# dnbaker/dashing2

Hardware: AMD Instinct MI355X
Metric: all-pairs sketch comparison throughput (pairs/s) (higher is better)
Workload: dtype u64

## Files before the change

dashing2_amd/capi.py:

```python
import ctypes as C
import os
import subprocess

import numpy as np

_HERE = os.path.dirname(os.path.abspath(__file__))
LIB_PATH = os.environ.get("D2G_LIB") or os.path.join(_HERE, "libd2g.so")
_lib = None

SIMILARITY, CONTAINMENT, SYMMETRIC_CONTAINMENT, POISSON_LLR, INTERSECTION, UNION_SIZE = range(6)
CMP_AUTO, CMP_DIRECT, CMP_BITSLICE, CMP_PLANES = 0, 1, 2, 3
BITSLICE_OPS_PER_GROUP_EXTRA = 1


TIME_K1, TIME_K2, TIME_K2PREP, TIME_K3, TIME_K0 = 2, 4, 8, 16, 32
TIME_KNN = 64
TIME_DEDUP = 128
TIME_FILTER = 256
TIME_KSET = 512
TIME_SCREEN = 1024


class D2GError(RuntimeError):
    def __init__(self, status, detail=""):
        self.status = status
        name = lib().d2g_strerror(status).decode() if _lib is not None else str(status)
        super().__init__(f"d2g error {status} ({name}){': ' + detail if detail else ''}")


def build(jobs=8):
    subprocess.check_call(["make", "-s", f"-j{jobs}", "-C", os.path.join(_HERE, "csrc")])
    return LIB_PATH

# ... 1323 lines not shown
                lib().d2g_cmp_set_destroy(self._h)
            self._h = None

    __del__ = close

    def export_operand_dev(self, planes_out_ptr, meta_out_ptr, stream=None):
        self.ctx._check(lib().d2g_cmp_set_export_operand_dev(self.ctx._h, self._h, planes_out_ptr, meta_out_ptr, stream))

    def update_dev(self, dev_ptr, stream=None):
        self.ctx._check(lib().d2g_cmp_set_update_dev(self.ctx._h, self._h, dev_ptr, stream))

    def status(self, stream=None):
        self.ctx._check(lib().d2g_cmp_set_status(self.ctx._h, self._h, stream))

    def sparse_info(self, stream=None):
        a = np.zeros(4, np.uint32)
        self.ctx._check(lib().d2g_cmp_set_sparse_info(self.ctx._h, self._h, stream, a.ctypes.data))
        return sparse_info_dict(a)

    def sparse_detail(self, stream=None):
        a = np.zeros(10, np.uint64)
        self.ctx._check(lib().d2g_cmp_set_sparse_detail(self.ctx._h, self._h, stream, a.ctypes.data))
        return {"looked": bool(a[0]), "looked_dense": bool(a[1]), "entries": int(a[2]), "family_pairs": int(a[3]), "shared_values": int(a[4]),
                "planes": int(a[5]), "binned": bool(a[6]), "bin_cshift": int(a[7]), "schedule": "merged" if a[8] else "classic", "prepare_kernels": int(a[9])}

    def fill_detail(self):
        a = np.zeros(4, np.uint64)
        self.ctx._check(lib().d2g_cmp_set_fill_detail(self.ctx._h, self._h, a.ctypes.data))
        return {"announced": int(a[0]), "rank": int(a[1]), "riders": int(a[2]), "launch": int(a[3])}

    def debug_pairs(self, cap=1 << 24, stream=None):
        buf = np.empty(cap, np.uint64)
        roots = np.empty(self.N, np.uint32)
        n = _sz()
        self.ctx._check(lib().d2g_cmp_set_debug_pairs(self.ctx._h, self._h, stream, buf.ctypes.data, cap, C.byref(n), roots.ctypes.data))
        e = buf[:n.value]
        e = e[e != np.uint64(0xFFFFFFFFFFFFFFFF)]
        return np.stack([(e & np.uint64(0xFFFFFFFF)).astype(np.uint32), (e >> np.uint64(32)).astype(np.uint32)], axis=1), roots

    def planes(self, stream=None):
        md, nb, mean = C.c_uint(), _int(), _f32()
        self.ctx._check(lib().d2g_cmp_set_planes(self.ctx._h, self._h, stream, C.byref(md), C.byref(nb), C.byref(mean)))
        return int(md.value), int(nb.value), float(mean.value)

    def eqcount_ut_dev(self, out_dev_ptr, r0=0, r1=None, stream=None):
        r1 = self.N if r1 is None else r1
        self.ctx._check(lib().d2g_cmp_eqcount_ut_dev(self.ctx._h, self._h, r0, r1, out_dev_ptr, stream))
# ... 260 lines not shown
```

dashing2_amd/csrc/d2g_internal.h:

```cpp
#pragma once
#include "../../include/d2g.h"
#include <hip/hip_runtime.h>
#include <cstdio>
#include <memory>
#include <string>
#include <utility>

#include <vector>
struct d2g_ctx;
int d2g_hip_status(d2g_ctx *ctx, hipError_t e, const char *what);

template <class T, bool Pinned> class d2g_owned {
    T *p_ = nullptr; size_t cap_ = 0;
public:
    d2g_owned() = default;
    d2g_owned(d2g_owned &&o) noexcept : p_(o.p_), cap_(o.cap_) { o.p_ = nullptr; o.cap_ = 0; }
    d2g_owned &operator=(d2g_owned &&o) noexcept { if (this != &o) { reset(); p_ = o.p_; cap_ = o.cap_; o.p_ = nullptr; o.cap_ = 0; } return *this; }
    ~d2g_owned() { reset(); }
    void reset() { if (p_) (void)(Pinned ? hipHostFree(p_) : hipFree(p_)); p_ = nullptr; cap_ = 0; }
    int alloc(d2g_ctx *ctx, size_t n, const char *what, unsigned flags = hipHostMallocDefault) {
        reset();
        const hipError_t e = Pinned ? hipHostMalloc((void **)&p_, n * sizeof(T), flags) : hipMalloc((void **)&p_, n * sizeof(T));
        if (e != hipSuccess) p_ = nullptr; else cap_ = n;
        return d2g_hip_status(ctx, e, what);
// ... 27 lines not shown
};

struct d2g_evlog {
    std::vector<d2g_event> a, b;
};

struct d2g_tuning {
    std::vector<std::pair<std::string, std::string>> kv;
    const char *get(const char *name) const {
        for (const auto &p : kv) if (p.first == name) return p.second.c_str();
        return nullptr;
    }
};
void d2g_tuning_load(d2g_tuning &t);
struct d2g_k2_tuning {
    bool sparse = true;
    size_t min_n = 8192;
    int link = 1;
    double tile_frac = 0.35;
    int olink = 1;
    int emit_big = 0;
    int ride = 127;
    int rank_share = 35;
    int merge = 1;
    int remember = 1;
    size_t long_list = 786432;
    int predict = 1;
    int list_form = 0;
    size_t list_div = 8;
    bool sort = true;
    int tagbits_max = 31;
    int id16 = 1;
    int nsplit_req = 0;
};
d2g_k2_tuning d2g_k2_tuning_resolve(const d2g_tuning &t);
std::string d2g_k2_tuning_json(const d2g_ctx *ctx);
uint64_t d2g_k2_tuning_hash(const d2g_ctx *ctx);

constexpr int K3_MAXBBITS = 12;
constexpr int K3_ROUND_KEYS = 1400;
constexpr int K3_TARGET = 1024;
constexpr int K3_L1BITS = 8;
constexpr uint64_t K3_SPLIT_MIN = 4 * 1400;
struct d2g_k3_tuning {
    bool compact = false;
    bool light = true;
    uint32_t l1bits = K3_L1BITS;
// ... 91 lines not shown
```

dashing2_amd/csrc/d2g_k2.h:

```cpp
#pragma once
#include "d2g_internal.h"

#include <algorithm>

struct SpRider { uint32_t *out; size_t cnt; const uint32_t *vsrc; uint32_t vimm, own, piece0; };
constexpr SpRider SP_NO_RIDER{nullptr, 0, nullptr, 0u, 0xFFFFFFFFu, 0u};
constexpr int SP_FILL_PER_THREAD = 8, SP_FILL_THREADS = 256;
inline size_t sp_fill_pieces(size_t cnt) { return div_up<size_t>(cnt / 4 + 1, (size_t)SP_FILL_THREADS * SP_FILL_PER_THREAD); }
#ifndef D2G_SP_RW_M_LINK0
#define D2G_SP_RW_M_LINK0 8
#endif
#ifndef D2G_SP_RW_M_PLANES
#define D2G_SP_RW_M_PLANES 5
#endif
constexpr unsigned SP_RW_PLAN = 6, SP_RW_FLATTEN = 5, SP_RW_COUNT = 5, SP_RW_ATTACH = 5, SP_RW_SCAN = 8, SP_RW_ALL = 35;
constexpr unsigned SP_RW_M_LINK0 = D2G_SP_RW_M_LINK0, SP_RW_M_PLANES = D2G_SP_RW_M_PLANES;
constexpr int BS_RANK_THREADS = 1024, BS_RANK_PF = 12;
constexpr uint32_t SP_RANK_FILL_PER_WG = (uint32_t)(BS_RANK_PF * BS_RANK_THREADS * 16 / (SP_FILL_THREADS * SP_FILL_PER_THREAD * 16));
static_assert(SP_RANK_FILL_PER_WG * SP_FILL_THREADS * SP_FILL_PER_THREAD == BS_RANK_PF * BS_RANK_THREADS, "the rank kernel's stores of one workgroup are whole pieces");

struct SpInit {
    uint32_t *label = nullptr, *ones = nullptr, *zero = nullptr;
    uint32_t n = 0, owords = 0, zwords = 0;
};
// ... 37 lines not shown
        next += n;
        *grid = own + n;
        return r;
    }
};

struct SpFilled {
    uint32_t *out = nullptr;
    size_t cnt = 0;
    size_t pieces = 0;
    const uint32_t *src = nullptr;
    bool by_riders = false;
    void set_early(uint32_t *o, size_t n, const uint32_t *s) { out = o; cnt = n; pieces = (size_t)-1; src = s; by_riders = false; }
    void set_by_riders(const SpAnnounced &a) { out = a.out; cnt = a.cnt; pieces = a.next; src = a.vsrc; by_riders = true; }
    size_t done_for(const uint32_t *o, size_t n, const uint32_t *s, size_t npieces) const { return (out == o && cnt == n && src == s) ? std::min(pieces, npieces) : 0; }
    void void_after_prepare() { if (by_riders) out = nullptr; }
    void clear() { out = nullptr; }
};

enum SpMappedWord : uint32_t { SP_MW_GAVEUP = 0, SP_MW_LIST_LEN = 1, SP_MW_SUMS = 2, SP_MW_TICKET = 6, SP_MW_WORDS = 16 };

struct SpDecision {
    unsigned prepares = 0; bool skipped = false;
    bool merged = false; unsigned kernels = 0;
    int skip_cached = -1;
    bool sample_pending = false; uint32_t sample_ticket = 0;
    bool pred_valid = false, pred_dense = false; double pred_entries = 0, pred_family_pairs = 0;
    bool big = true;
    bool looked = false, looked_dense = false; uint32_t samp_sums[4] = {0, 0, 0, 0};
    uint64_t fill_announced = 0, fill_rank = 0, fill_carried = 0;
};

struct SpState {
    unsigned sp_launch = 0;
    d2g_dev<uint32_t> d_stream_s;
    d2g_dev<uint32_t> d_sperm;
    d2g_dev<uint32_t> d_sinv;
    d2g_dev<uint32_t> d_label;
    d2g_dev<uint32_t> d_owner;
    size_t owner_stride = 0;
    d2g_dev<uint32_t> d_segend;
    d2g_dev<uint32_t> d_posseg;
    d2g_dev<uint32_t> d_hint;
    d2g_dev<uint32_t> d_spz;
    size_t spz_words = 0;
    uint32_t *d_lcnt = nullptr;
    uint32_t *d_gbm = nullptr;
// ... 97 lines not shown
```

dashing2_amd/csrc/d2g_k2_bitslice.hip:

```cpp
#include "d2g_internal.h"
#include "d2g_k2.h"
#include "d2g_k2_shape.h"
#include <chrono>
#include <cstring>
#include <algorithm>
#include <vector>

namespace {

typedef uint32_t u32x16 __attribute__((ext_vector_type(16)));
typedef u32x16 __attribute__((aligned(4))) u32x16_u;
constexpr uint32_t BS_EMPTY = 0xFFFFFFFFu;

constexpr uint32_t BS_DUP = 0x80000000u;
constexpr uint32_t BS_UNIQ = 0x80000000u;
constexpr uint32_t BS_PENDING = 0x40000000u;
constexpr int BS_LOG_TLDS_MAX = 15;
template <typename IdT> struct BsId;
template <> struct BsId<uint32_t> { static constexpr uint32_t UNIQ = BS_UNIQ; static constexpr int UBIT = 31; };
template <> struct BsId<uint16_t> { static constexpr uint32_t UNIQ = 0x8000u; static constexpr int UBIT = 15; };
constexpr size_t BS_ID16_MAX_N = ((size_t(1) << BS_LOG_TLDS_MAX) * 2) / 3;
static_assert(BS_ID16_MAX_N / 2 < BsId<uint16_t>::UNIQ, "16-bit ids: the highest rank (N / 2) must stay below the unique flag");
static_assert((size_t(1) << BS_LOG_TLDS_MAX) - 1 <= 0xFFFFu, "16-bit ids: the general single-partition kernel parks a table slot in ids[] between its two loops");

// ... 437 lines not shown
        uint32_t mx = 0;
        for (uint32_t x = 0; x < 32; ++x) mx = max(mx, d2s[perm_s[(uint32_t)g * 32 + x]]);
        meta[g] = mx + 1;
        if (ex_meta) ex_meta[g] = mx + 1;
    }
}

__global__ __launch_bounds__(BS_PLAN_THREADS) void bs_colplan_kernel(BsPlanArgs pa, SpRider rider) {
    SP_RIDE_OR_WORK(rider);
    extern __shared__ __attribute__((aligned(16))) uint32_t plan_lds[];
    bs_colplan_body<BS_PLAN_THREADS>(pa, bs_plan_lds(plan_lds, (uint32_t)pa.ntb * 32u));
}

constexpr int BS_FORM_STREAM = 1, BS_FORM_EXCHANGE = 2;
constexpr size_t BS_SLACK = 64;
struct BsPlanesArgs {
    const void *ids; size_t N, Npad; uint32_t *planes, *stream; size_t Nstride; int nbits_cap; const uint32_t *meta; int forms;
    const uint32_t *perm, *colcnt, *sperm;
};
BsPlanesArgs planes_args_of(const d2g_cmp_set *set, uint32_t *planes, int forms) {
    return BsPlanesArgs{set->d_ids.get(), set->N, set->Npad, planes, set->d_stream, set->Nstride, set->nbits_cap, set->d_meta, forms, set->d_perm, set->d_colcnt, nullptr};
}
template <bool SPLIT, typename IdT = uint32_t>
__device__ __forceinline__ void bs_planes_body(const BsPlanesArgs &a, size_t bx, size_t tb) {
    static_assert(!SPLIT || sizeof(IdT) == 4, "bs_planes_body: split ranks are 32-bit ids");
    constexpr int UBIT = BsId<IdT>::UBIT;
    const IdT *__restrict__ ids = static_cast<const IdT *>(a.ids);
    const uint32_t *__restrict__ meta = a.meta, *__restrict__ perm = a.perm, *__restrict__ colcnt = a.colcnt, *__restrict__ sperm = a.sperm;
    uint32_t *__restrict__ planes = a.planes, *__restrict__ stream = a.stream;
    const size_t N = a.N, Npad = a.Npad, Nstride = a.Nstride;
    const int nbits_cap = a.nbits_cap, forms = a.forms;
    const size_t jpos = bx * 256 + threadIdx.x;
    const size_t slot = (forms & BS_FORM_STREAM) ? stream_slot_wave(meta, (int)tb) : 0;
    if (jpos >= Nstride) return;
    const size_t j = sperm ? (size_t)sperm[jpos] : jpos;
    const int nbits = live_planes(meta, (int)tb);
    typedef const u32x16_u __attribute__((address_space(4))) *slots_ptr;
    const u32x16_u pa = *(slots_ptr)(uintptr_t)(perm + tb * 32), pb = *(slots_ptr)(uintptr_t)(perm + tb * 32 + 16);
    uint32_t id[32];
#pragma unroll
    for (int x = 0; x < 32; ++x) {
        const uint32_t t = x < 16 ? pa[x] : pb[x - 16];
        const bool real = t != BS_NOCOL && j < N;
        uint32_t w = real ? ids[(size_t)t * Npad + j] : 0u;
        if (SPLIT && real && !(w >> 31)) w = (w & BS_RANK_MASK) + colcnt[(size_t)t * BS_CC_STRIDE + (w >> BS_SPLIT_SHIFT)];
        id[x] = w;
    }
    uint32_t u = 0;
#pragma unroll
    for (int x = 0; x < 32; ++x) u |= (id[x] >> UBIT) << x;
    uint32_t *dst = planes + tb * (size_t)(nbits_cap + 1) * Nstride + jpos;
    const bool ex = forms & BS_FORM_EXCHANGE, st = forms & BS_FORM_STREAM;
    uint32_t *sdst = st ? stream + slot * 2 * Nstride + jpos : nullptr;
    for (int b = 0; b < nbits; ++b) {
        uint32_t w = 0;
// ... 307 lines not shown
        const int logTl = set->logT < BS_LOG_TLDS_MAX ? set->logT : BS_LOG_TLDS_MAX;
        const size_t lds = (size_t(1) << logTl) * sizeof(uint32_t);
        const bool id16 = set->id_bits == 16;
        D2G_CHECK(ctx, !(multi && id16), "bitslice: the multi-partition rank kernel with 16-bit ids");
        void (*kern)(const uint64_t *, size_t, size_t, uint32_t, int, void *, uint32_t *, uint32_t *, int, uint32_t, int, uint32_t *, size_t, SpRider, uint32_t) = bs_rank_kernel<false, false>;
        const bool fast = !multi && N <= (size_t)BS_RANK_PF * BS_RANK_THREADS;
        if (multi) kern = bs_rank_kernel<true, false>;
        else if (fast) kern = id16 ? bs_rank_kernel<false, true, uint16_t> : bs_rank_kernel<false, true>;
        else if (id16) kern = bs_rank_kernel<false, false, uint16_t>;
        if (lds > 48 * 1024)
            D2G_HIP(ctx, hipFuncSetAttribute((const void *)kern, hipFuncAttributeMaxDynamicSharedMemorySize, (int)lds));
        if (nsplit > 1) D2G_HIP(ctx, hipMemsetAsync(set->d_ids, 0, S * Npad * sizeof(uint32_t), s));
        const bool look = sparse_path && sp_sample_due(ctx, set);
        SpRider rank_fill = SP_NO_RIDER; uint32_t rank_n = 0;
        if (sparse_path && fast && !look && sp->announced.riding() < SP_SIDE_FILL_PIECES)
            rank_fill = sp->announced.take_first((unsigned)ctx->k2.rank_share, (uint64_t)SP_RANK_FILL_PER_WG * S, &rank_n);
        D2G_CHECK(ctx, rank_n <= (uint64_t)SP_RANK_FILL_PER_WG * S * nsplit, "bitslice: the rank kernel's share of the fill does not fit its grid");
        if (sp) sp->dec.fill_rank = rank_n;
        hipLaunchKernelGGL(kern, dim3((unsigned)(S * nsplit)), dim3(BS_RANK_THREADS), lds, s, set->d_cols, N, Npad, set->T, set->logT,
                           (void *)set->d_ids.get(), set->d_colcnt, set->d_meta + set->ntb, ctx->k2.tagbits_max, (uint32_t)S, nsplit,
                           (sp && nsplit == 1) ? sp->d_owner.get() : (uint32_t *)nullptr, sp ? sp->owner_stride : 0, rank_fill, rank_n);
        if (sp) sp->dec.kernels = 2 + (join.ev ? 1 : 0);
        if (look) { if (int rc = sp_sample_enqueue(ctx, set, s)) return rc; if (sp->dec.sample_pending) sp->dec.kernels += 2; }
        const bool merged = sparse_path && !look && ctx->k2.merge && nsplit == 1 && sp->d_owner && ctx->k2.olink && ctx->k2.link && sp->dec.skip_cached != 1;
        if (sp) sp->dec.merged = merged;
        if (!merged) {
            unsigned g = 1; const SpRider rd = sp ? sp->announced.take(1, SP_RW_PLAN, false, 1, &g) : SP_NO_RIDER;
            const BsPlanArgs pa{set->d_colcnt, (uint32_t)S, set->ntb, nsplit, set->d_perm, set->d_meta, set->d_meta + set->ntb, set->ex_meta, set->ex_status, ctx->k2.sort ? 1 : 0};
            hipLaunchKernelGGL(bs_colplan_kernel, dim3(g), dim3(BS_PLAN_THREADS), bs_plan_lds_words((uint32_t)set->ntb * 32u, pa.sort) * 4, s, pa, rd);
            if (sp) sp->dec.kernels += 1;
        }
    }
    if (sparse_path) {
        if (!sp->dec.merged) { if (int rc = launch_planes(ctx, set, set->d_planes, BS_FORM_STREAM, s)) return rc; sp->dec.kernels += 1; }
        if (int rc = sp_sample_collect(ctx, set, s)) return rc;
        if (int rc = sp_prepare_order(ctx, set, nsplit > 1, s)) return rc;
        if (int rc = sp_permute(ctx, set, s)) return rc;
        set->srt_valid = true; set->nat_valid = true;
        sp->dec.fill_carried = sp->announced.next - sp->dec.fill_rank;
        if (sp->announced.riding()) sp->filled.set_by_riders(sp->announced);
        else sp->filled.void_after_prepare();
        sp->announced.served();
        D2G_HIP(ctx, hipGetLastError());
        return D2G_OK;
    }
    if (sp) sp->announced.served();
    const int forms = set->export_only ? BS_FORM_EXCHANGE : (BS_FORM_STREAM | (set->want_exchange ? BS_FORM_EXCHANGE : 0));
// ... 95 lines not shown
                      hipStream_t s) {
    return launch_bitslice(ctx, set, rect_shape(set->N, a0, a1, b0, b1), StoreEq{eq_out}, s);
}

int d2g_bitslice_managed_sparse_alloc(d2g_ctx *ctx, d2g_cmp_set *set) {
    if (!set->borrowed || set->sparse_ok()) return D2G_OK;
    set->ncols = (size_t)set->ntb * 32;
    if (!(sparse_enabled(ctx, set->N) && set->S < 65536)) return D2G_OK;
    const char *what = "bitslice sparse alloc";
    if (set->d_ids.alloc(ctx, set->ncols * set->Npad, what) != D2G_OK ||
        set->d_colcnt.alloc(ctx, set->ncols * BS_CC_STRIDE, what) != D2G_OK ||
        hipMemset(set->d_colcnt, 0, set->ncols * BS_CC_STRIDE * sizeof(uint32_t)) != hipSuccess) {
        set->d_ids.reset(); set->d_colcnt.reset();
        (void)hipGetLastError();
        return D2G_OK;
    }
    if (sp_alloc(ctx, set) != D2G_OK) (void)hipGetLastError();
    return D2G_OK;
}

int d2g_bitslice_managed_ready(d2g_ctx *ctx, d2g_cmp_set *set, hipStream_t s) {
    if (!set->borrowed || !set->sparse_ok()) return D2G_OK;
    dim3 grid((unsigned)div_up<size_t>(set->Npad, 256), (unsigned)set->ntb);
    set->sp->dec.merged = false; set->sp->dec.kernels = 1;
    hipLaunchKernelGGL(sp_unpack_kernel, grid, dim3(256), 0, s, set->d_planes, set->Nstride, set->nbits_cap, set->d_meta, set->N, set->Npad, set->d_ids, set->d_colcnt, sp_init_of(set));
    if (int rc = sp_prepare_order(ctx, set, false, s)) return rc;
    if (int rc = sp_permute(ctx, set, s)) return rc;
    D2G_HIP(ctx, hipGetLastError());
    set->srt_valid = true;
    return D2G_OK;
}

void d2g_bitslice_forget(d2g_cmp_set *set) {
    if (!set->sp) return;
    if (set->sp->h_gaveup) { set->sp->h_gaveup[SP_MW_GAVEUP] = 0; set->sp->h_gaveup[SP_MW_LIST_LEN] = 0; }
    set->sp->dec.prepares = 0; set->sp->dec.pred_valid = false;
}

int d2g_bitslice_sparse_info(d2g_ctx *ctx, const d2g_cmp_set *set, hipStream_t s, uint32_t *out4) {
    out4[0] = out4[1] = out4[2] = out4[3] = 0;
    if (!set->srt_valid || !set->sp) { D2G_HIP(ctx, hipStreamSynchronize(s)); return D2G_OK; }
    const SpState &sp = *set->sp;
    uint32_t c[4] = {0, 0, 0, 0}, ord[4] = {0, 0, 0, 0}, pl = 0;
    if (!sp.last_ctl) { D2G_HIP(ctx, hipStreamSynchronize(s)); out4[0] = 1; return D2G_OK; }
    D2G_HIP(ctx, hipMemcpyAsync(c, sp.last_ctl, sizeof c, hipMemcpyDeviceToHost, s));
    D2G_HIP(ctx, hipMemcpyAsync(ord, sp.d_order, sizeof ord, hipMemcpyDeviceToHost, s));
    D2G_HIP(ctx, hipMemcpyAsync(&pl, sp.d_plctl, sizeof pl, hipMemcpyDeviceToHost, s));
    D2G_HIP(ctx, hipStreamSynchronize(s));
    const bool dense = (c[1] & 1u) || (size_t)c[0] * 5 > (size_t)c[3] * 2;
    out4[0] = 1; out4[1] = c[0]; out4[2] = (ord[0] ? 1u : 0u) | (dense ? 2u : 4u) | (ord[0] ? 8u : 0u) | (sp.dec.skipped ? 16u : 0u);
    out4[3] = ord[0] ? 0u : (uint32_t)std::min<size_t>(pl, sp.plist_cap);
    return D2G_OK;
}

int d2g_bitslice_sparse_detail(d2g_ctx *ctx, const d2g_cmp_set *set, hipStream_t s, uint64_t *out8) {
    uint32_t binned = 0;
    if (set->sp) D2G_HIP(ctx, hipMemcpyAsync(&binned, set->sp->d_plctl + SP_PL_BINNED, 4, hipMemcpyDeviceToHost, s));
    D2G_HIP(ctx, hipStreamSynchronize(s));
    if (!set->sp) return D2G_OK;
    const SpState &sp = *set->sp;
    out8[0] = sp.dec.looked ? 1 : 0; out8[1] = sp.dec.looked_dense ? 1 : 0;
    if (sp.dec.looked) for (int x = 0; x < 4; ++x) out8[2 + x] = sp.dec.samp_sums[x];
    out8[6] = binned ? 1 : 0; out8[7] = sp.bin_cshift;
    out8[8] = sp.dec.merged ? 1 : 0; out8[9] = sp.dec.kernels;
    return D2G_OK;
}

void d2g_bitslice_fill_detail(const d2g_cmp_set *set, uint64_t *out4) {
    out4[0] = out4[1] = out4[2] = out4[3] = 0;
    if (!set->sp) return;
    const SpDecision &d = set->sp->dec;
    out4[0] = d.fill_announced; out4[1] = d.fill_rank; out4[2] = d.fill_carried; out4[3] = d.fill_announced - d.fill_rank - d.fill_carried;
}

int d2g_sparse_bin_geometry(size_t N, uint32_t *cshift, uint32_t *nch, uint32_t *nbins, int *binned_ok) {
    if (!N) return D2G_ERR_INVALID;
    const SpBinGeom g = sp_bin_geometry(N);
    if (cshift) *cshift = g.cshift;
    if (nch) *nch = g.nch;
    if (nbins) *nbins = g.nbins;
    if (binned_ok) *binned_ok = g.ok ? 1 : 0;
    return D2G_OK;
}

int d2g_bitslice_debug_read(d2g_ctx *ctx, const d2g_cmp_set *set, hipStream_t s, uint64_t *pairs_out, size_t cap, size_t *npairs, uint32_t *root_out ) {
    *npairs = 0;
    if (!set->srt_valid || !set->sp) { D2G_HIP(ctx, hipStreamSynchronize(s)); return D2G_OK; }
// ... 45 lines not shown
```

dashing2_amd/csrc/d2g_k2_sparse.h:

```cpp
constexpr uint32_t SP_NONE = 0xFFFFFFFFu;
constexpr uint32_t SP_SAMPLE_ROWS = 16, SP_SAMPLE_FAM = 4, SP_SAMPLE_COLS = 32;
constexpr unsigned long long SP_NULL_ENTRY = ~0ull;
#ifndef D2G_SP_KS
#define D2G_SP_KS 8
#endif
#ifndef D2G_SP_WPE
#define D2G_SP_WPE 8
#endif

template <typename IdT = uint32_t>
__device__ __forceinline__ uint32_t sp_rank(uint32_t w, const uint32_t *__restrict__ colcnt, size_t t, bool split) {
    if ((w >> BsId<IdT>::UBIT) || w == 0) return 0;
    if constexpr (sizeof(IdT) == 2) return w;
    else return split ? (w & BS_RANK_MASK) + colcnt[t * BS_CC_STRIDE + (w >> BS_SPLIT_SHIFT)] : w;
}

__device__ __forceinline__ uint32_t sp_ld(const uint32_t *p) { return __hip_atomic_load(p, __ATOMIC_RELAXED, __HIP_MEMORY_SCOPE_AGENT); }

__device__ __forceinline__ uint32_t sp_find(uint32_t *label, uint32_t l) {
    for (int h = 0; h < 64; ++h) {
        const uint32_t p = sp_ld(&label[l]);
        if (p == l) break;
        const uint32_t g = sp_ld(&label[p]);
        if (g != p) label[l] = g;
// ... 331 lines not shown
    const int first = __ffsll((long long)m) - 1;
    uint32_t base = 0;
    if (lane == first) base = atomicAdd(&cnt[lead], (uint32_t)__popcll(m));
    base = __shfl(base, first);
    if (live && r == lead) p = base + (uint32_t)__popcll(m & ((1ull << lane) - 1));
    else if (live) p = atomicAdd(&cnt[r], 1u);
    if (live) { sperm[p] = (uint32_t)j; sinv[j] = p; posseg[p] = uint2{seg_start[r], seg_end[r]}; }
}

struct SpColWork { uint32_t *ents; uint4 *vals; uint32_t ecap, vcap; };
__device__ __forceinline__ unsigned long long *sp_pl_streams(uint32_t *plctl) { return reinterpret_cast<unsigned long long *>(plctl + 8 + (((uintptr_t)(plctl + 8) >> 2) & 1u)); }
__device__ __forceinline__ unsigned long long *sp_pl_proj(uint32_t *plctl) { return reinterpret_cast<unsigned long long *>(plctl + 1 + (((uintptr_t)(plctl + 1) >> 2) & 1u)); }

#ifndef D2G_SP_EMIT_T
#define D2G_SP_EMIT_T 512
#endif
#ifdef D2G_SP_TRACE
__device__ unsigned long long g_emit_trace[4096 * 16];
#define EM_STAMP(k) do { if (threadIdx.x == 0 && blockIdx.x < 4096 && lo == 0) g_emit_trace[blockIdx.x * 16 + (k)] = __builtin_amdgcn_s_memrealtime(); } while (0)
#else
#define EM_STAMP(k) do { } while (0)
#endif
constexpr uint32_t SP_EMIT_VCAP = 1536, SP_EMIT_ECAP = 32768, SP_EMIT_T = D2G_SP_EMIT_T;
template <typename IdT = uint32_t>
__global__ __launch_bounds__(SP_EMIT_T) __attribute__((amdgpu_waves_per_eu(8, 8))) void sp_emit_kernel(const void *__restrict__ ids_void, size_t N, size_t Npad, uint32_t ncols, const uint32_t *__restrict__ colcnt, int split,
                                                            const uint32_t *__restrict__ seg, uint32_t *__restrict__ order,
                                                            SpColWork cw, uint32_t *__restrict__ plctl, uint32_t plcap, uint32_t *__restrict__ gaveup, int big) {
    __shared__ uint32_t first[SP_EMIT_VCAP];
    __shared__ uint32_t cnt[SP_EMIT_VCAP];
    __shared__ uint32_t mrec[SP_EMIT_VCAP];
    __shared__ uint32_t vpre[SP_EMIT_VCAP];
    __shared__ uint32_t second[SP_EMIT_VCAP];
    __shared__ uint32_t cntb[SP_EMIT_VCAP];
    __shared__ unsigned long long wave_tot64[16];
    __shared__ uint32_t s_base, s_ebase, s_vbase, s_stop, s_cut, s_nent, s_nm;
    if (order[0]) return;
    constexpr uint32_t T = SP_EMIT_T, PER = (SP_EMIT_VCAP + T - 1) / T;
    const uint32_t tid = threadIdx.x;
    const size_t t = blockIdx.x;
    const uint32_t d2 = colcnt[t * BS_CC_STRIDE + 4];
    if (d2 == 0) return;
    const IdT *__restrict__ col = static_cast<const IdT *>(ids_void) + t * Npad;
    const uint32_t n32 = (uint32_t)N;
    auto for_each_holder = [&](auto &&fn) {
        if constexpr (sizeof(IdT) == 2) {
            typedef uint32_t u32x2 __attribute__((ext_vector_type(2)));
#pragma unroll 1
            for (uint32_t j0 = 0; j0 < n32; j0 += T * 8) {
                uint32_t w[4];
                u32x2 sg[4];
// ... 983 lines not shown
    }
    const double scale = (double)N / (2.0 * SP_SAMPLE_ROWS), pairs = (double)N * (double)(N - 1) / 2.0;
    sp.dec.pred_valid = true;
    for (int x = 0; x < 4; ++x) sp.dec.samp_sums[x] = h[x];
    sp.dec.pred_entries = (double)h[0] * scale;
    sp.dec.pred_family_pairs = (double)h[1] * scale;
    const double values = (double)h[2], planes = set->ncols ? (double)h[3] / (double)set->ncols : 1.0;
    const double g = (double)set->ntb / 32.0, per_pair = 0.002 + 0.00094 * planes * g;
    const double dense_ns = pairs * per_pair, sparse_ns = (3.0 + 3.6 * g) * (double)N + 0.055 * sp.dec.pred_entries + 0.077 * values + 9.0 * per_pair * sp.dec.pred_family_pairs;
    sp.dec.pred_dense = sp.dec.pred_entries > (double)sp.plist_cap || sparse_ns > 0.97 * dense_ns;
    sp.h_gaveup[SP_MW_GAVEUP] = sp.dec.pred_dense ? 1u : 0u;
    return D2G_OK;
}

int sp_launch_merged(d2g_ctx *ctx, d2g_cmp_set *set, const SpOlinkArgs *l0, unsigned nx, unsigned npair, unsigned nflat, hipStream_t s) {
    SpState &sp = *set->sp;
    const BsPlanArgs pa{set->d_colcnt, (uint32_t)set->S, set->ntb, 1, set->d_perm, set->d_meta, set->d_meta + set->ntb, set->ex_meta, set->ex_status, ctx->k2.sort ? 1 : 0};
    const bool id16 = set->id_bits == 16;
    const size_t nlink = (size_t)nx * npair, gx = div_up<size_t>(set->Nstride, 256), nplanes = gx * (size_t)set->ntb;
    D2G_CHECK(ctx, 1 + nlink < 0x40000000u && nflat + nplanes < 0x40000000u, "bitslice sparse: a merged launch does not fit a grid");
    unsigned g;
    SpRider rd = sp.announced.take((unsigned)(1 + nlink), SP_RW_M_LINK0, false, 1, &g);
    hipLaunchKernelGGL((id16 ? sp_link0_plan_kernel<uint16_t> : sp_link0_plan_kernel<uint32_t>), dim3(g), dim3(256), bs_plan_lds_words((uint32_t)set->ntb * 32u, pa.sort) * 4, s, pa, l0 ? *l0 : SpOlinkArgs{}, (uint32_t)nx, rd);
    rd = sp.announced.take((unsigned)(nflat + nplanes), SP_RW_M_PLANES, false, 2, &g);
    hipLaunchKernelGGL((id16 ? bs_planes_flatten_kernel<uint16_t> : bs_planes_flatten_kernel<uint32_t>), dim3(g), dim3(256), 0, s, planes_args_of(set, set->d_planes, BS_FORM_STREAM), (uint32_t)gx, (uint32_t)nflat, sp.d_label.get(), rd);
    sp.dec.kernels += 2;
    D2G_HIP(ctx, hipGetLastError());
    return D2G_OK;
}

int sp_prepare_order(d2g_ctx *ctx, d2g_cmp_set *set, bool split, hipStream_t s) {
    const size_t N = set->N, Npad = set->Npad, S = set->ncols;
    SpState &sp = *set->sp;
    const bool remembered = sp.dec.skip_cached >= 0 ? sp.dec.skip_cached == 1 : sp_will_skip(ctx, sp);
    sp.dec.skip_cached = -1;
    const bool skip = sp.dec.pred_valid ? sp.dec.pred_dense : (remembered && sp.announced.riding() == 0);
    sp.dec.big = sp_expect_long_list(ctx, sp);
    ++sp.dec.prepares;
    sp.dec.looked = sp.dec.pred_valid; sp.dec.looked_dense = sp.dec.pred_valid && sp.dec.pred_dense;
    sp.dec.pred_valid = false;
    D2G_CHECK(ctx, !(skip && sp.dec.merged), "bitslice sparse: the merged schedule was chosen for a prepare that skips the ordering");
    if (skip) {
        ++sp.dec.kernels;
        hipLaunchKernelGGL(sp_giveup_kernel, dim3(1), dim3(64), 0, s, sp.d_order, sp.d_fullctl, (uint32_t)std::min<size_t>(sp_full_candidates(Npad), 0xFFFFFFFFu));
        D2G_HIP(ctx, hipGetLastError());
        sp.dec.skipped = true;
        return D2G_OK;
    }
    sp.dec.skipped = false;
// ... 27 lines not shown
            { unsigned g; const SpRider rd = sp.announced.take(nb, SP_RW_FLATTEN, false, 2, &g); hipLaunchKernelGGL(sp_flatten_kernel, dim3(g), dim3(256), 0, s, la, N, rd); }
            hipLaunchKernelGGL(link1, dim3(div_up<unsigned>(npair, ustride)), dim3(1024), (size_t)cap * 8, s, ids, N, Npad, (uint32_t)S, set->d_colcnt, split ? 1 : 0, cap, ustride,
                               la, sp.d_hint);
            sp.dec.kernels += 3;
        }
    } else if (sp.dec.merged) {
        if (int rc = sp_launch_merged(ctx, set, nullptr, 0, 0, 0, s)) return rc;
    }
    const size_t ntile_all = (Npad / 32) * (Npad / BS_CB);
    const uint32_t seg_limit = (uint32_t)std::min<size_t>((size_t)((double)ntile_all * tu.tile_frac), 0x3FFFFFFF);
    sp.dec.kernels += 4 + ((tu.link && S >= 2) ? 1 : 0) + (sp.dec.big ? 1 : 0);
    { unsigned g; const SpRider rd = sp.announced.take(nb, SP_RW_COUNT, false, 4, &g); hipLaunchKernelGGL(sp_count_kernel, dim3(g), dim3(256), 0, s, la, lb, N, sp.d_lcnt, sp.d_order, rd); }
    if (tu.link && S >= 2) {
        unsigned g; const SpRider rd = sp.announced.take(nb, SP_RW_ATTACH, false, 8, &g);
        hipLaunchKernelGGL(sp_attach_kernel, dim3(g), dim3(256), 0, s, lb, sp.d_lcnt, sp.d_hint, N, Npad, sp.d_order, rd);
    }
    const uint32_t CW = (uint32_t)((Npad / BS_CB + 31) / 32);
    { unsigned g; const SpRider rd = sp.announced.take(1, SP_RW_SCAN, false, 16, &g);
      hipLaunchKernelGGL(sp_scan_kernel, dim3(g), dim3(1024), 0, s, sp.d_lcnt, N, sp.d_order, la, sp.d_segend, seg_limit, sp.d_gaveup, rd); }
    { unsigned g; const SpRider rd = sp.announced.take((unsigned)div_up<size_t>(set->Nstride, 256), 0, true, 32, &g);
      hipLaunchKernelGGL(sp_place_kernel, dim3(g), dim3(256), 0, s, lb, N, set->Nstride, sp.d_lcnt, sp.d_sperm, sp.d_sinv, sp.d_order,
                         la, sp.d_segend, CW, sp.d_gbm + 8, reinterpret_cast<uint2 *>(sp.d_posseg.get()), rd); }
    const SpColWork cw = sp_colwork_of(sp);
    hipLaunchKernelGGL((id16 ? sp_emit_kernel<uint16_t> : sp_emit_kernel<uint32_t>), dim3((unsigned)S), dim3(SP_EMIT_T), 0, s, ids, N, Npad, (uint32_t)S, set->d_colcnt, split ? 1 : 0, lb, sp.d_order,
                       cw, sp.d_plctl, (uint32_t)std::min<size_t>(sp.plist_cap, 0xFFFFFFFFu), sp.d_gaveup, (N >= 65536 || tu.emit_big) ? 1 : 0);
    if (sp.dec.big) hipLaunchKernelGGL(sp_pairs_kernel, dim3((unsigned)ctx->num_cus * 8), dim3(256), 0, s, sp_pairs_of(sp, cw, lb));
    D2G_HIP(ctx, hipGetLastError());
    return D2G_OK;
}

SpBins sp_bins_of(const SpState &sp) { return SpBins{sp.d_binc, sp.d_bstart, sp.nbins, sp.bin_nch, sp.bin_cshift}; }

int sp_permute(d2g_ctx *ctx, d2g_cmp_set *set, hipStream_t s) {
    SpState &sp = *set->sp;
    if (sp.dec.skipped) { sp.full_list_valid = true; return D2G_OK; }
    const size_t nrb = set->Npad / 32, ncb = set->Npad / BS_CB, ntile = nrb * ncb;
    const bool both = set->Nstride * 8 <= 156 * 1024;
    constexpr size_t LDS_PART = 128 * 1024;
    const uint32_t H = both ? 1u : (uint32_t)div_up<size_t>(set->Nstride * 4, LDS_PART);
    const uint32_t part = (uint32_t)(div_up<size_t>(div_up<size_t>(set->Nstride, H), 4) * 4);
    SpFullList fl{sp.d_gbm + 8, (uint32_t)nrb, (uint32_t)ncb, (uint32_t)((ncb + 31) / 32), sp.d_tiles_full, (uint32_t)sp.tiles_cap, sp.d_fullctl,
                  (uint32_t)std::min<size_t>(sp_full_candidates(set->Npad), 0xFFFFFFFFu), (uint32_t)div_up<size_t>(ntile, 1024), (uint32_t)set->N,
                  reinterpret_cast<const uint2 *>(sp.d_posseg.get())};
    const size_t nperm = (size_t)set->ntb * set->nbits_cap * (both ? 1 : 2) * H;
    const uint32_t plcap = (uint32_t)std::min<size_t>(sp.plist_cap, 0xFFFFFFFFu);
    SpHist hs{sp.d_plist, sp.d_plctl, plcap, sp.dec.big ? sp.bin_nwg : (uint32_t)ctx->num_cus, sp_bins_of(sp), sp.d_hoff, sp.dec.big ? 1 : 0,
              sp.h_gaveup ? sp.d_gaveup + SP_MW_LIST_LEN : nullptr};
    sp.full_list_valid = nperm + fl.nwg + hs.nhw < 0x7FFFFFFFu;
// ... 115 lines not shown
```

dashing2_amd/csrc/d2g_runtime.hip:

```cpp
#include "d2g_internal.h"
#include <algorithm>
#include <cstdlib>
#include <cstring>
#include <new>

static const char *const kTuningNames[] = {
    "D2G_BS_SORT", "D2G_BS_NSPLIT", "D2G_BS_TAGBITS", "D2G_BS_ID16", "D2G_K2_MERGE",
    "D2G_BS_SPARSE", "D2G_BS_SPARSE_MIN_N", "D2G_SP_LINK", "D2G_SP_TILE_FRAC", "D2G_SP_LIST_DIV", "D2G_SP_LONG_LIST", "D2G_SP_LIST_FORM", "D2G_SP_PREDICT", "D2G_SP_REMEMBER", "D2G_SP_EMIT_BIG", "D2G_SP_OLINK", "D2G_SP_RIDE", "D2G_SP_RANK_SHARE",
    "D2G_MGPU_CHUNKS",
    "D2G_K3_COMPACT", "D2G_K3_L1BITS", "D2G_K3_BUCKET_KEYS", "D2G_K3_SUB_KEYS", "D2G_K3_SPLIT_MIN", "D2G_K3_SUBBATCH", "D2G_K3_ROUND_KEYS",
    "D2G_K3_GUESS_SCALE", "D2G_K3_GRID_PER_CU", "D2G_K3_LIGHT", "D2G_K3_GQ_SCALE",
    "D2G_K3S_RANGE_KEYS", "D2G_KSET_SPLIT", "D2G_KSET_PBITS",
    "D2G_CS_TABLE_BYTES", "D2G_CS_LDS_CELLS",
};
void d2g_tuning_load(d2g_tuning &t) {
    t.kv.clear();
    for (const char *n : kTuningNames)
        if (const char *v = std::getenv(n)) t.kv.emplace_back(n, v);
}

d2g_k2_tuning d2g_k2_tuning_resolve(const d2g_tuning &t) {
    d2g_k2_tuning v;
    if (const char *e = t.get("D2G_BS_SPARSE")) v.sparse = !(e[0] == '0');
    if (const char *e = t.get("D2G_BS_SPARSE_MIN_N")) v.min_n = (size_t)std::atoll(e);
    if (const char *e = t.get("D2G_SP_LINK")) v.link = std::atoi(e) != 0;
    if (const char *e = t.get("D2G_SP_TILE_FRAC")) { const double f = std::atof(e); if (f > 0 && f <= 1) v.tile_frac = f; }
    if (const char *e = t.get("D2G_SP_OLINK")) v.olink = std::atoi(e) != 0;
    if (const char *e = t.get("D2G_K2_MERGE")) v.merge = std::atoi(e) != 0;
    if (const char *e = t.get("D2G_SP_EMIT_BIG")) v.emit_big = std::atoi(e) != 0;
    if (const char *e = t.get("D2G_SP_REMEMBER")) v.remember = std::atoi(e) != 0;
    if (const char *e = t.get("D2G_SP_RIDE")) v.ride = std::atoi(e) & 127;
    if (const char *e = t.get("D2G_SP_RANK_SHARE")) { const int d = std::atoi(e); if (d >= 0 && d <= 35) v.rank_share = d; }
    if (const char *e = t.get("D2G_SP_LONG_LIST")) { const long long d = std::atoll(e); if (d >= 0) v.long_list = (size_t)d; }
    if (const char *e = t.get("D2G_SP_PREDICT")) v.predict = std::atoi(e) != 0;
    if (const char *e = t.get("D2G_SP_LIST_FORM")) { const int d = std::atoi(e); if (d >= 0 && d <= 2) v.list_form = d; }
    if (const char *e = t.get("D2G_SP_LIST_DIV")) { const long d = std::atol(e); if (d >= 1 && d <= (1 << 20)) v.list_div = (size_t)d; }
    if (const char *e = t.get("D2G_BS_SORT")) v.sort = !(e[0] == '0');
    if (const char *e = t.get("D2G_BS_TAGBITS")) { const int d = std::atoi(e); if (d >= 0 && d < 31) v.tagbits_max = d; }
    if (const char *e = t.get("D2G_BS_ID16")) v.id16 = std::atoi(e) != 0;
    if (const char *e = t.get("D2G_BS_NSPLIT")) { const int d = std::atoi(e); if (d == 1 || d == 2 || d == 4) v.nsplit_req = d; }
    return v;
}

d2g_k3_tuning d2g_k3_tuning_resolve(const d2g_tuning &t) {
    d2g_k3_tuning v;
    if (const char *e = t.get("D2G_K3_COMPACT")) v.compact = e[0] == '1';
    if (const char *e = t.get("D2G_K3_LIGHT")) v.light = !(e[0] == '0');
    if (const char *e = t.get("D2G_K3_L1BITS")) { const int d = std::atoi(e); if (d >= 0 && d <= K3_MAXBBITS) v.l1bits = (uint32_t)d; }
    if (const char *e = t.get("D2G_K3_BUCKET_KEYS")) { const long d = std::atol(e); if (d >= 1) v.bucket_keys = (uint64_t)d; }
    if (const char *e = t.get("D2G_K3_SUB_KEYS")) { const long d = std::atol(e); if (d >= 1) v.sub_keys = (uint64_t)d; }
    if (const char *e = t.get("D2G_K3_SPLIT_MIN")) { const long d = std::atol(e); if (d >= 1) v.split_min = (uint64_t)d; }
// ... 226 lines not shown
```

Baseline: 214.9 billion.

## Fuse bitslice planes build into sparse emit kernel launch as default schedule

Adds a third K2 merge schedule, now the default, in which the planes-building work is appended as extra blocks of the sparse emit kernel. The previous combined planes+flatten kernel is reduced to a flatten-only launch. Each extra 512-thread block handles two 256-thread planes items. The aim is to overlap planes construction with emit work and save a launch and a serialization point. The cost is a heterogeneous grid whose planes blocks run with the emit kernel's launch bounds and occupancy settings. It also adds the requirement that the non-split grid fits.

```diff
diff --git a/dashing2_amd/capi.py b/dashing2_amd/capi.py
--- a/dashing2_amd/capi.py
+++ b/dashing2_amd/capi.py
@@ -9,6 +9,7 @@
 _lib = None
 
 SIMILARITY, CONTAINMENT, SYMMETRIC_CONTAINMENT, POISSON_LLR, INTERSECTION, UNION_SIZE = range(6)
+K2_SCHEDULES = ("classic", "merged", "planes-emit")
 CMP_AUTO, CMP_DIRECT, CMP_BITSLICE, CMP_PLANES = 0, 1, 2, 3
 BITSLICE_OPS_PER_GROUP_EXTRA = 1
 
@@ -1378,7 +1379,7 @@
         a = np.zeros(10, np.uint64)
         self.ctx._check(lib().d2g_cmp_set_sparse_detail(self.ctx._h, self._h, stream, a.ctypes.data))
         return {"looked": bool(a[0]), "looked_dense": bool(a[1]), "entries": int(a[2]), "family_pairs": int(a[3]), "shared_values": int(a[4]),
-                "planes": int(a[5]), "binned": bool(a[6]), "bin_cshift": int(a[7]), "schedule": "merged" if a[8] else "classic", "prepare_kernels": int(a[9])}
+                "planes": int(a[5]), "binned": bool(a[6]), "bin_cshift": int(a[7]), "schedule": K2_SCHEDULES[min(int(a[8]), 2)], "merge": int(a[8]), "prepare_kernels": int(a[9])}
 
     def fill_detail(self):
         a = np.zeros(4, np.uint64)
diff --git a/dashing2_amd/csrc/d2g_internal.h b/dashing2_amd/csrc/d2g_internal.h
--- a/dashing2_amd/csrc/d2g_internal.h
+++ b/dashing2_amd/csrc/d2g_internal.h
@@ -73,7 +73,7 @@
     int emit_big = 0;
     int ride = 127;
     int rank_share = 35;
-    int merge = 1;
+    int merge = 2;
     int remember = 1;
     size_t long_list = 786432;
     int predict = 1;
diff --git a/dashing2_amd/csrc/d2g_k2.h b/dashing2_amd/csrc/d2g_k2.h
--- a/dashing2_amd/csrc/d2g_k2.h
+++ b/dashing2_amd/csrc/d2g_k2.h
@@ -83,7 +83,7 @@
 
 struct SpDecision {
     unsigned prepares = 0; bool skipped = false;
-    bool merged = false; unsigned kernels = 0;
+    int merged = 0; unsigned kernels = 0;
     int skip_cached = -1;
     bool sample_pending = false; uint32_t sample_ticket = 0;
     bool pred_valid = false, pred_dense = false; double pred_entries = 0, pred_family_pairs = 0;
diff --git a/dashing2_amd/csrc/d2g_k2_bitslice.hip b/dashing2_amd/csrc/d2g_k2_bitslice.hip
--- a/dashing2_amd/csrc/d2g_k2_bitslice.hip
+++ b/dashing2_amd/csrc/d2g_k2_bitslice.hip
@@ -483,7 +483,7 @@
     return BsPlanesArgs{set->d_ids.get(), set->N, set->Npad, planes, set->d_stream, set->Nstride, set->nbits_cap, set->d_meta, forms, set->d_perm, set->d_colcnt, nullptr};
 }
 template <bool SPLIT, typename IdT = uint32_t>
-__device__ __forceinline__ void bs_planes_body(const BsPlanesArgs &a, size_t bx, size_t tb) {
+__device__ __forceinline__ void bs_planes_body(const BsPlanesArgs &a, size_t bx, size_t tb, uint32_t tid = threadIdx.x) {
     static_assert(!SPLIT || sizeof(IdT) == 4, "bs_planes_body: split ranks are 32-bit ids");
     constexpr int UBIT = BsId<IdT>::UBIT;
     const IdT *__restrict__ ids = static_cast<const IdT *>(a.ids);
@@ -491,7 +491,7 @@
     uint32_t *__restrict__ planes = a.planes, *__restrict__ stream = a.stream;
     const size_t N = a.N, Npad = a.Npad, Nstride = a.Nstride;
     const int nbits_cap = a.nbits_cap, forms = a.forms;
-    const size_t jpos = bx * 256 + threadIdx.x;
+    const size_t jpos = bx * 256 + tid;
     const size_t slot = (forms & BS_FORM_STREAM) ? stream_slot_wave(meta, (int)tb) : 0;
     if (jpos >= Nstride) return;
     const size_t j = sperm ? (size_t)sperm[jpos] : jpos;
@@ -845,7 +845,7 @@
                            (sp && nsplit == 1) ? sp->d_owner.get() : (uint32_t *)nullptr, sp ? sp->owner_stride : 0, rank_fill, rank_n);
         if (sp) sp->dec.kernels = 2 + (join.ev ? 1 : 0);
         if (look) { if (int rc = sp_sample_enqueue(ctx, set, s)) return rc; if (sp->dec.sample_pending) sp->dec.kernels += 2; }
-        const bool merged = sparse_path && !look && ctx->k2.merge && nsplit == 1 && sp->d_owner && ctx->k2.olink && ctx->k2.link && sp->dec.skip_cached != 1;
+        const int merged = (sparse_path && !look && ctx->k2.merge && nsplit == 1 && sp->d_owner && ctx->k2.olink && ctx->k2.link && sp->dec.skip_cached != 1) ? ctx->k2.merge : 0;
         if (sp) sp->dec.merged = merged;
         if (!merged) {
             unsigned g = 1; const SpRider rd = sp ? sp->announced.take(1, SP_RW_PLAN, false, 1, &g) : SP_NO_RIDER;
@@ -987,7 +987,7 @@
 int d2g_bitslice_managed_ready(d2g_ctx *ctx, d2g_cmp_set *set, hipStream_t s) {
     if (!set->borrowed || !set->sparse_ok()) return D2G_OK;
     dim3 grid((unsigned)div_up<size_t>(set->Npad, 256), (unsigned)set->ntb);
-    set->sp->dec.merged = false; set->sp->dec.kernels = 1;
+    set->sp->dec.merged = 0; set->sp->dec.kernels = 1;
     hipLaunchKernelGGL(sp_unpack_kernel, grid, dim3(256), 0, s, set->d_planes, set->Nstride, set->nbits_cap, set->d_meta, set->N, set->Npad, set->d_ids, set->d_colcnt, sp_init_of(set));
     if (int rc = sp_prepare_order(ctx, set, false, s)) return rc;
     if (int rc = sp_permute(ctx, set, s)) return rc;
@@ -1027,7 +1027,7 @@
     out8[0] = sp.dec.looked ? 1 : 0; out8[1] = sp.dec.looked_dense ? 1 : 0;
     if (sp.dec.looked) for (int x = 0; x < 4; ++x) out8[2 + x] = sp.dec.samp_sums[x];
     out8[6] = binned ? 1 : 0; out8[7] = sp.bin_cshift;
-    out8[8] = sp.dec.merged ? 1 : 0; out8[9] = sp.dec.kernels;
+    out8[8] = (uint64_t)sp.dec.merged; out8[9] = sp.dec.kernels;
     return D2G_OK;
 }
 
diff --git a/dashing2_amd/csrc/d2g_k2_sparse.h b/dashing2_amd/csrc/d2g_k2_sparse.h
--- a/dashing2_amd/csrc/d2g_k2_sparse.h
+++ b/dashing2_amd/csrc/d2g_k2_sparse.h
@@ -377,10 +377,24 @@
 #define EM_STAMP(k) do { } while (0)
 #endif
 constexpr uint32_t SP_EMIT_VCAP = 1536, SP_EMIT_ECAP = 32768, SP_EMIT_T = D2G_SP_EMIT_T;
-template <typename IdT = uint32_t>
+template <typename IdT = uint32_t, bool PLANES = false>
 __global__ __launch_bounds__(SP_EMIT_T) __attribute__((amdgpu_waves_per_eu(8, 8))) void sp_emit_kernel(const void *__restrict__ ids_void, size_t N, size_t Npad, uint32_t ncols, const uint32_t *__restrict__ colcnt, int split,
                                                             const uint32_t *__restrict__ seg, uint32_t *__restrict__ order,
-                                                            SpColWork cw, uint32_t *__restrict__ plctl, uint32_t plcap, uint32_t *__restrict__ gaveup, int big) {
+                                                            SpColWork cw, uint32_t *__restrict__ plctl, uint32_t plcap, uint32_t *__restrict__ gaveup, int big,
+                                                            BsPlanesArgs pl, uint32_t gx, uint32_t nitems) {
+    if constexpr (PLANES) {
+        if (blockIdx.x >= ncols) {
+            const uint32_t item = (blockIdx.x - ncols) * 2u + (uint32_t)__builtin_amdgcn_readfirstlane((int)(threadIdx.x >> 8));
+#ifdef D2G_SP_TRACE
+            if ((threadIdx.x & 255u) == 0 && blockIdx.x < 4096) g_emit_trace[blockIdx.x * 16 + (threadIdx.x >> 8)] = __builtin_amdgcn_s_memrealtime();
+#endif
+            if (item < nitems) bs_planes_body<false, IdT>(pl, item % gx, item / gx, threadIdx.x & 255u);
+#ifdef D2G_SP_TRACE
+            if ((threadIdx.x & 255u) == 0 && blockIdx.x < 4096) g_emit_trace[blockIdx.x * 16 + 2 + (threadIdx.x >> 8)] = __builtin_amdgcn_s_memrealtime();
+#endif
+            return;
+        }
+    }
     __shared__ uint32_t first[SP_EMIT_VCAP];
     __shared__ uint32_t cnt[SP_EMIT_VCAP];
     __shared__ uint32_t mrec[SP_EMIT_VCAP];
@@ -1410,9 +1424,14 @@
     unsigned g;
     SpRider rd = sp.announced.take((unsigned)(1 + nlink), SP_RW_M_LINK0, false, 1, &g);
     hipLaunchKernelGGL((id16 ? sp_link0_plan_kernel<uint16_t> : sp_link0_plan_kernel<uint32_t>), dim3(g), dim3(256), bs_plan_lds_words((uint32_t)set->ntb * 32u, pa.sort) * 4, s, pa, l0 ? *l0 : SpOlinkArgs{}, (uint32_t)nx, rd);
-    rd = sp.announced.take((unsigned)(nflat + nplanes), SP_RW_M_PLANES, false, 2, &g);
-    hipLaunchKernelGGL((id16 ? bs_planes_flatten_kernel<uint16_t> : bs_planes_flatten_kernel<uint32_t>), dim3(g), dim3(256), 0, s, planes_args_of(set, set->d_planes, BS_FORM_STREAM), (uint32_t)gx, (uint32_t)nflat, sp.d_label.get(), rd);
-    sp.dec.kernels += 2;
+    if (sp.dec.merged == 2) {
+        if (nflat) { rd = sp.announced.take(nflat, SP_RW_M_PLANES, false, 2, &g); hipLaunchKernelGGL(sp_flatten_kernel, dim3(g), dim3(256), 0, s, sp.d_label.get(), set->N, rd); }
+        sp.dec.kernels += nflat ? 2 : 1;
+    } else {
+        rd = sp.announced.take((unsigned)(nflat + nplanes), SP_RW_M_PLANES, false, 2, &g);
+        hipLaunchKernelGGL((id16 ? bs_planes_flatten_kernel<uint16_t> : bs_planes_flatten_kernel<uint32_t>), dim3(g), dim3(256), 0, s, planes_args_of(set, set->d_planes, BS_FORM_STREAM), (uint32_t)gx, (uint32_t)nflat, sp.d_label.get(), rd);
+        sp.dec.kernels += 2;
+    }
     D2G_HIP(ctx, hipGetLastError());
     return D2G_OK;
 }
@@ -1486,8 +1505,16 @@
       hipLaunchKernelGGL(sp_place_kernel, dim3(g), dim3(256), 0, s, lb, N, set->Nstride, sp.d_lcnt, sp.d_sperm, sp.d_sinv, sp.d_order,
                          la, sp.d_segend, CW, sp.d_gbm + 8, reinterpret_cast<uint2 *>(sp.d_posseg.get()), rd); }
     const SpColWork cw = sp_colwork_of(sp);
+    if (sp.dec.merged == 2) {
+        static_assert(SP_EMIT_T == 512, "sp_emit_kernel<IdT, true>: a block takes two 256-thread planes items");
+        const size_t gx = div_up<size_t>(set->Nstride, 256), nitems = gx * (size_t)set->ntb;
+        D2G_CHECK(ctx, !split && S + div_up<size_t>(nitems, 2) < 0x40000000u, "bitslice sparse: the emit + planes launch does not fit a grid");
+        hipLaunchKernelGGL((id16 ? sp_emit_kernel<uint16_t, true> : sp_emit_kernel<uint32_t, true>), dim3((unsigned)(S + div_up<size_t>(nitems, 2))), dim3(SP_EMIT_T), 0, s, ids, N, Npad, (uint32_t)S, set->d_colcnt, 0, lb, sp.d_order,
+                           cw, sp.d_plctl, (uint32_t)std::min<size_t>(sp.plist_cap, 0xFFFFFFFFu), sp.d_gaveup, (N >= 65536 || tu.emit_big) ? 1 : 0,
+                           planes_args_of(set, set->d_planes, BS_FORM_STREAM), (uint32_t)gx, (uint32_t)nitems);
+    } else
     hipLaunchKernelGGL((id16 ? sp_emit_kernel<uint16_t> : sp_emit_kernel<uint32_t>), dim3((unsigned)S), dim3(SP_EMIT_T), 0, s, ids, N, Npad, (uint32_t)S, set->d_colcnt, split ? 1 : 0, lb, sp.d_order,
-                       cw, sp.d_plctl, (uint32_t)std::min<size_t>(sp.plist_cap, 0xFFFFFFFFu), sp.d_gaveup, (N >= 65536 || tu.emit_big) ? 1 : 0);
+                       cw, sp.d_plctl, (uint32_t)std::min<size_t>(sp.plist_cap, 0xFFFFFFFFu), sp.d_gaveup, (N >= 65536 || tu.emit_big) ? 1 : 0, BsPlanesArgs{}, 0u, 0u);
     if (sp.dec.big) hipLaunchKernelGGL(sp_pairs_kernel, dim3((unsigned)ctx->num_cus * 8), dim3(256), 0, s, sp_pairs_of(sp, cw, lb));
     D2G_HIP(ctx, hipGetLastError());
     return D2G_OK;
diff --git a/dashing2_amd/csrc/d2g_runtime.hip b/dashing2_amd/csrc/d2g_runtime.hip
--- a/dashing2_amd/csrc/d2g_runtime.hip
+++ b/dashing2_amd/csrc/d2g_runtime.hip
@@ -26,7 +26,7 @@
     if (const char *e = t.get("D2G_SP_LINK")) v.link = std::atoi(e) != 0;
     if (const char *e = t.get("D2G_SP_TILE_FRAC")) { const double f = std::atof(e); if (f > 0 && f <= 1) v.tile_frac = f; }
     if (const char *e = t.get("D2G_SP_OLINK")) v.olink = std::atoi(e) != 0;
-    if (const char *e = t.get("D2G_K2_MERGE")) v.merge = std::atoi(e) != 0;
+    if (const char *e = t.get("D2G_K2_MERGE")) { const int d = std::atoi(e); v.merge = d <= 0 ? 0 : d >= 2 ? 2 : 1; }
     if (const char *e = t.get("D2G_SP_EMIT_BIG")) v.emit_big = std::atoi(e) != 0;
     if (const char *e = t.get("D2G_SP_REMEMBER")) v.remember = std::atoi(e) != 0;
     if (const char *e = t.get("D2G_SP_RIDE")) v.ride = std::atoi(e) & 127;
```

New measurement: 219.4 billion (median of 6 runs). 1.02x the previous value.
